# zhiqwang/yolort

Hardware: NVIDIA H100
Metric: images/sec end-to-end (letterbox->NMS) (higher is better)
Workload: dtype f16

## Files before the change

### include/yolort_b200.h

```cpp
#ifndef YOLORT_B200_H
#define YOLORT_B200_H

#include <stddef.h>
#include <stdint.h>

#ifdef __cplusplus
extern "C" {
#endif

#define YB_OK 0
#define YB_ERR_INVALID (-1)
#define YB_ERR_CUDA (-2)
#define YB_ERR_WORKSPACE (-3)

#define YB_U8 0
#define YB_F16 1
#define YB_BF16 2
#define YB_F32 3
#define YB_F8E4M3 4

const char* yb_last_error(void);
int yb_abi_version(void);

typedef struct {
// ... 45 lines not shown
  int32_t level_start;
  int32_t anchors_per_image;
  float stride_px;
  float anchors_px[8];
  float score_thresh;
  int64_t cap_per_image;
  uint64_t* keys;
  void* boxes;
  int32_t* img_count;
  int32_t* img_maxc;
} yb_head_decode;

typedef struct {
  const void* weight;
  const float* bias;
  int32_t Cout, Cout_pad, K_pad;
  int32_t act;
  void* out;
  int32_t out_cstride;
  int32_t own_C;
  const void* extra;
  int32_t extra_C, extra_cstride;
  int32_t store_first;
} yb_conv_chain;

typedef struct {
  int32_t kind;
  int32_t dtype;
  int32_t N, H, W;
  int32_t Cin, in_cstride;
  const void* in;
  int32_t Ho, Wo;
  int32_t Cout, out_cstride;
  void* out;
  int32_t ksize, stride, pad;
  int32_t act;
  const void* weight;
  int32_t Cin_pad, Cout_pad;
  const float* bias;
  const void* residual;
  int32_t res_cstride;
  int32_t reserved;
  const yb_head_decode* decode;
  const yb_conv_chain* chain;
} yb_op_desc;

#define YB_CONV_FORCE_IM2COL 1
#define YB_CONV_BAND_STEM 2
#define YB_CONV_FORCE_PLANES 4
#define YB_CONV_NO_NSPLIT 8
#define YB_CONV_ONE_CTA 16
#define YB_CONV_NO_TAIL_SPLIT 64
#define YB_CONV_PAIR_N64 128
#define YB_CONV_E4M3_F16_OUT 16
#define YB_CONV_E4M3_BF16_OUT 32

int yb_conv_chain_supported(const yb_op_desc* op);

#define YB_CONV_KERNEL_IM2COL 0
#define YB_CONV_KERNEL_PATCH 1
#define YB_CONV_KERNEL_E4M3 2
#define YB_CONV_TILING_ROWS 0
#define YB_CONV_TILING_CLASSIC 1
#define YB_CONV_TILING_WRAP 2
#define YB_CONV_TILING_STRIDE2 3
typedef struct {
  int32_t kernel;
  int32_t block_n;
  int32_t n_tiles;
  int32_t weights_resident;
  int32_t tiles_per_pass;
  int32_t slots;
  int32_t ring;
  int32_t store_cols;
  int32_t store_bufs;
  int32_t groups;
  int32_t resident_ctas;
  int32_t chained;
  int32_t smem_bytes;
  int32_t grid;
  int32_t tiling;
  int32_t m_tiles;
  int32_t work_items;
  int32_t tail_n;
  int32_t tail_tiles;
  int32_t tail_split;
} yb_conv_info;

int yb_conv_config(const yb_op_desc* op, yb_conv_info* info);

typedef struct yb_plan yb_plan;

int yb_plan_create(const yb_op_desc* ops, int n_ops, yb_plan** plan_out);
int yb_plan_run(yb_plan* plan, void* stream);
int yb_plan_run_range(yb_plan* plan, int first, int count, void* stream);
int yb_plan_num_launches(const yb_plan* plan);
int yb_plan_destroy(yb_plan* plan);

#define YB_MAX_LEVELS 4
#define YB_MAX_ANCHORS 4

typedef struct {
  const void* logits;
  int32_t dtype;
  int32_t H, W;
  int64_t stride_n, stride_a, stride_y, stride_x;
// ... 365 lines not shown
```

### yolort_b200/_C.py

```python
import ctypes
import itertools
import math
import os
from typing import Dict, List, Optional, Sequence, Tuple

import torch

_HERE = os.path.dirname(os.path.abspath(__file__))
LIB_PATH = os.environ.get("YB_LIB_PATH") or os.path.join(_HERE, "libyolort_b200.so")

YB_U8, YB_F16, YB_BF16, YB_F32, YB_F8E4M3 = 0, 1, 2, 3, 4
YB_LAYOUT_NCHW, YB_LAYOUT_S2D16 = 0, 1
YB_OP_CONV, YB_OP_SPP_POOL, YB_OP_UPSAMPLE2X, YB_OP_ATTENTION, YB_OP_DWCONV, YB_OP_SE, YB_OP_AVGPOOL = 0, 1, 2, 3, 4, 5, 6
YB_OP_QUANTIZE = 7
YB_ACT_NONE, YB_ACT_SILU, YB_ACT_HARDSWISH, YB_ACT_LEAKY01, YB_ACT_RELU = 0, 1, 2, 3, 4
YB_CONV_FORCE_IM2COL, YB_CONV_BAND_STEM, YB_CONV_FORCE_PLANES, YB_CONV_NO_NSPLIT, YB_CONV_ONE_CTA = 1, 2, 4, 8, 16
YB_CONV_NO_TAIL_SPLIT = 64
YB_CONV_PAIR_N64 = 128
YB_CONV_E4M3_F16_OUT, YB_CONV_E4M3_BF16_OUT = 16, 32
YB_CONV_KERNEL_IM2COL, YB_CONV_KERNEL_PATCH, YB_CONV_KERNEL_E4M3 = 0, 1, 2
PATCH_TILINGS = {1: "classic", 2: "wrap", 3: "stride2"}
YB_MAX_LEVELS, YB_MAX_ANCHORS = 4, 4
NMS_TV_AUTO, NMS_EXACT_PER_CLASS, NMS_OFFSET_TRICK = 0, 1, 2

EXPORTED_SYMBOLS = (
    "yb_last_error",
    "yb_abi_version",
    "yb_letterbox_geometry",
    "yb_letterbox",
    "yb_letterbox_strided",
    "yb_canvas_rescale",
    "yb_scale_coords_params",
    "yb_conv_chain_supported",
    "yb_conv_config",
    "yb_plan_create",
    "yb_plan_run",
    "yb_plan_run_range",
    "yb_plan_num_launches",
    "yb_plan_destroy",
    "yb_decode_nms_workspace_bytes",
    "yb_decode_nms_debug_offset",
    "yb_decode_nms",
    "yb_decode_dense",
    "yb_decode_nms_tta_workspace_bytes",
    "yb_decode_nms_tta",
    "yb_nms_layout",
    "yb_nms_begin",
    "yb_nms_finish",
    "yb_decode_candidates",
    "yb_batched_nms_workspace_bytes",
    "yb_batched_nms",
    "yb_jpeg_parse",
    "yb_jpeg_workspace_bytes",
    "yb_jpeg_decode",
    "yb_coco_append",
    "yb_coco_evaluate_workspace_bytes",
    "yb_coco_evaluate",
    "yb_yolo_loss_workspace_bytes",
    "yb_yolo_loss_layout",
    "yb_yolo_loss_forward",
    "yb_yolo_loss_backward",
    "yb_augment_prepare",
    "yb_augment",
    "yb_augment_sample",
    "yb_v5_augment_prepare",
    "yb_v5_augment",
    "yb_v5_mixup",
    "yb_v5_resize_prepare",
    "yb_v5_resize",
    "yb_v5_compose_prepare",
    "yb_v5_compose",
# ... 1331 lines not shown
```

### yolort_b200/csrc/conv3x3_patch_sm90.cu

```cuda
#include <cstdlib>

#include "common.cuh"
#include "conv_epilogue.cuh"
#include "conv_chain.cuh"
#include "conv_sm90.h"

namespace yb {
namespace {

constexpr int kMaxA = 4, kMaxB = 12;
constexpr int kConsumers = 2;
constexpr int kThreads = 128 * (1 + kConsumers);
constexpr int kStageBufBytes = 128 * 128;
constexpr int kMaxBlockN = 128;
constexpr size_t kSmemBudget = 216 * 1024;
constexpr size_t kStaticSmem = (2 * kMaxA + 2 * kMaxB + 2) * 8 + 2 * kMaxBlockN * 4;
constexpr uint32_t kConsumerBar = 1;

struct TileGeom {
  int tile_h, tile_w;
  int x_step;
  int pitch, patch_h;
  int gpr;
  int sbo_rows;
  int alloc_rows;
};

struct PatchParams {
  int N, H, W;
  int tiles_x, tiles_y, m_tiles, n_tiles, num_tasks;
  int block_n, block_k, chunks;
  int a_slots, b_stages, b_resident;
  int pair;
  int s2;
  int band;
  int ctas;
  int store_cols, store_bufs, bias_len;
  int stage_buf_bytes;
  int kk_last;
  TileGeom tg;
  uint32_t a_bytes, a_stride, b_sub_bytes, b_res_bytes;
  const float* bias;
  EpilogueParams ep;
  ChainParams ch;
};

__device__ __forceinline__ void tma_load_tiled_4d(const void* desc, uint64_t* bar, void* smem_dst, int c, int w,
                                                  int h, int n) {
  asm volatile(
      "cp.async.bulk.tensor.4d.shared::cluster.global.mbarrier::complete_tx::bytes"
      " [%0], [%1, {%3, %4, %5, %6}], [%2];" ::"r"(smem_u32(smem_dst)),
      "l"(reinterpret_cast<uint64_t>(desc)), "r"(smem_u32(bar)), "r"(c), "r"(w), "r"(h), "r"(n)
      : "memory");
}
__device__ __forceinline__ void tma_load_tiled_5d(const void* desc, uint64_t* bar, void* smem_dst, int c, int par, int w,
                                                  int h, int n) {
  asm volatile(
      "cp.async.bulk.tensor.5d.shared::cluster.global.mbarrier::complete_tx::bytes"
      " [%0], [%1, {%3, %4, %5, %6, %7}], [%2];" ::"r"(smem_u32(smem_dst)),
      "l"(reinterpret_cast<uint64_t>(desc)), "r"(smem_u32(bar)), "r"(c), "r"(par), "r"(w), "r"(h), "r"(n)
      : "memory");
}
__device__ __forceinline__ void tma_store_4d(const void* desc, const void* smem_src, int c, int w, int h, int n) {
  asm volatile("cp.async.bulk.tensor.4d.global.shared::cta.bulk_group [%0, {%2, %3, %4, %5}], [%1];" ::"l"(
                   reinterpret_cast<uint64_t>(desc)),
               "r"(smem_u32(smem_src)), "r"(c), "r"(w), "r"(h), "r"(n)
               : "memory");
}

__device__ __forceinline__ void tile_coords(const PatchParams& p, int m_tile, int& n_img, int& y0, int& x0) {
  const int tpi = p.tiles_x * p.tiles_y;
  n_img = m_tile / tpi;
  const int t = m_tile - n_img * tpi;
  const int ty = t / p.tiles_x, tx = t - ty * p.tiles_x;
  y0 = ty * p.tg.tile_h;
  x0 = tx * p.tg.x_step;
}

__device__ __forceinline__ void consumer_sync() { named_bar_sync(kConsumerBar, 128 * kConsumers); }

template <bool kBf16, int kN, bool kPair>
__device__ __forceinline__ void issue_tap(int mode, int tap, int kc, bool first, float* acc, uint32_t a0, uint32_t a1,
                                          uint32_t a_hi, uint32_t b_lo, uint32_t b_hi) {
  for (int k = 0; k < kc; ++k) {
    const bool accum = !(first && k == 0);
    const uint64_t db = desc_lohi(b_lo + 2 * k, b_hi);
    if (mode == 2) {
      wgmma_mma<kBf16, kN>(acc, desc_lohi(((tap % 3) == 1 ? a0 : a1) + 2 * k, a_hi), db, accum);
    } else {
// ... 448 lines not shown
        mbar_wait(&b_full[sb], (kb / p.b_stages) & 1);
        const int dy = tap / 3, dx = tap - dy * 3;
        const uint32_t a_tap = a_lo + static_cast<uint32_t>(dy * p.tg.pitch + dx) * row16;
        const uint32_t b_lo = b_lo0 + static_cast<uint32_t>(sb) * b_step16;
        for (int k = 0; k < kc; ++k)
          wgmma_mma<kBf16, kN>(acc, desc_lohi(a_tap + 2 * k, a_hi), desc_lohi(b_lo + 2 * k, b_hi),
                               !(c == 0 && tap == 0 && k == 0));
        wgmma_commit();
        wgmma_wait<1>();
        if (wg_leader) {
          if (prev_sb >= 0) mbar_arrive(&b_empty[prev_sb]);
          if (prev_sa >= 0) mbar_arrive(&a_empty[prev_sa]);
        }
        prev_sb = sb;
        prev_sa = -1;
      }
      prev_sa = active ? sa : -1;
      ka += cnt;
    }
    wgmma_wait<0>();
    if (wg_leader) {
      mbar_arrive(&b_empty[prev_sb]);
      if (prev_sa >= 0) mbar_arrive(&a_empty[prev_sa]);
    }
    fence_acc<kN / 2>(acc);

    int n_img, y0, x0;
    tile_coords(p, m_first + team, n_img, y0, x0);
#pragma unroll
    for (int rr = 0; rr < 2; ++rr) {
      const int grp = fr.loc[rr] >> 3;
      const int yy = grp / p.tg.gpr, xx = (grp - yy * p.tg.gpr) * 8 + (fr.loc[rr] & 7);
      const int y = y0 + yy, x = x0 + xx;
      fr.ok[rr] = active && yy < p.tg.tile_h && y < p.H && x < p.W;
      fr.row[rr] = (static_cast<long long>(n_img) * p.H + y) * p.W + x;
    }
    uint8_t* team_staging = staging + static_cast<size_t>(team) * p.store_bufs * p.stage_buf_bytes;
#pragma unroll
    for (int c0 = 0; c0 < kN; c0 += 64, ++store_idx) {
      uint8_t* buf = team_staging + (store_idx & 1) * p.stage_buf_bytes;
      epilogue_box<kBf16, kN>(p.ep, acc, c0, 64, s_bias, fr, n0, buf, lane);
      fence_proxy_async_smem();
      if (issuer) tma_store_wait_read<0>();
      named_bar_sync(1 + team, 256);
      if (issuer) {
        if (active && n0 + c0 < p.ep.Cout) tma_store_4d(&tmap_out, buf, n0 + c0, x0, y0, n_img);
        tma_store_commit();
      }
    }
  }
  if (issuer) tma_store_wait_all<0>();
}

}

using PatchKernelFn = void (*)(const CUtensorMap, const CUtensorMap, const CUtensorMap, const CUtensorMap, const CUtensorMap,
                               const CUtensorMap, const PatchParams);

static bool quad_plan(const PatchParams& kp) { return kp.pair == 2 && !kp.s2 && kp.block_n == 128; }

template <bool kBf16>
PatchKernelFn select_patch_kernel_t(const PatchParams& kp) {
  if (quad_plan(kp)) return conv3x3_patch_quad_kernel<kBf16>;
  if (kp.ctas == 2) {
    if (kp.ch.on) return kp.block_n == 32 && kp.ch.n2 == 64 ? conv3x3_patch_kernel<kBf16, 32, 64, 2> : nullptr;
    switch (kp.block_n) {
      case 32: return conv3x3_patch_kernel<kBf16, 32, 0, 2>;
      case 64: return conv3x3_patch_kernel<kBf16, 64, 0, 2>;
      default: return nullptr;
    }
  }
  if (kp.ch.on) {
    if (kp.block_n == 32) return kp.ch.n2 == 64 ? conv3x3_patch_kernel<kBf16, 32, 64, 1> : conv3x3_patch_kernel<kBf16, 32, 128, 1>;
    return kp.ch.n2 == 64 ? conv3x3_patch_kernel<kBf16, 64, 64, 1> : conv3x3_patch_kernel<kBf16, 64, 128, 1>;
  }
  switch (kp.block_n) {
    case 32: return conv3x3_patch_kernel<kBf16, 32, 0, 1>;
    case 64: return conv3x3_patch_kernel<kBf16, 64, 0, 1>;
    default: return conv3x3_patch_kernel<kBf16, 128, 0, 1>;
  }
}
PatchKernelFn select_patch_kernel(const PatchParams& kp) {
  return kp.ep.is_bf16 ? select_patch_kernel_t<true>(kp) : select_patch_kernel_t<false>(kp);
}

namespace {
double classic_eff(int H, int W) {
  const int ty = (H + 15) / 16, tx = (W + 7) / 8;
  return static_cast<double>(H) * W / (static_cast<double>(ty) * tx * 128);
}
double wrap_eff(int H, int W) {
  if (W > 22 || W < 9) return 0.0;
  return static_cast<double>(H) * W / (static_cast<double>((H + 4) / 5) * 128);
}
TileGeom pick_geom(int H, int W, bool allow_wrap, bool s2) {
  TileGeom g;
  if (s2) {
    g.tile_h = 16; g.tile_w = 8; g.x_step = 8; g.pitch = 9; g.patch_h = 33; g.gpr = 1; g.sbo_rows = 18;
    g.alloc_rows = 33 * 9;
  } else if (allow_wrap && wrap_eff(H, W) > classic_eff(H, W)) {
    g.tile_h = 5; g.tile_w = 24; g.x_step = 24; g.pitch = 24; g.patch_h = 7; g.gpr = 3; g.sbo_rows = 8;
    g.alloc_rows = 8 * 24;
  } else {
    g.tile_h = 16; g.tile_w = 8; g.x_step = 8; g.pitch = 10; g.patch_h = 18; g.gpr = 1; g.sbo_rows = 10;
    g.alloc_rows = 18 * 10;
  }
  return g;
}
}

bool patch_conv_eligible(const yb_op_desc& d) {
  if (d.kind != YB_OP_CONV || d.ksize != 3 || d.pad != 1) return false;
  if (d.reserved & YB_CONV_FORCE_IM2COL) return false;
  if (d.stride == 2)
    return (d.reserved & YB_CONV_BAND_STEM) == 0 && d.W % 2 == 0 && d.H % 2 == 0 && classic_eff(d.Ho, d.Wo) >= 0.7 &&
           ((d.Cin <= 64 && d.Cout <= 128) || (d.reserved & YB_CONV_FORCE_PLANES));
// ... 80 lines not shown
        break;
      }
    }
  }
  const size_t avail_ns = budget - staging_ns - 1024 - chain_bytes;
  kp.pair = (!kp.b_resident && !kp.band && !kp.s2 && kp.m_tiles >= 2) ? 2 : 1;
  const int quad_tiles = d.Cout / 128;
  const int quad_tasks = ((kp.m_tiles + 1) / 2) * quad_tiles;
  const int grid_q = quad_tasks < sms ? quad_tasks : sms;
  const bool quad = ctas == 1 && kp.pair == 2 && d.chain == nullptr && d.Cout % 128 == 0 &&
                    !(d.reserved & YB_CONV_PAIR_N64) && grid_q % quad_tiles == 0 && quad_tasks >= sms &&
                    2 * ((quad_tasks + sms - 1) / sms) <= (2 * quad_tasks + sms - 1) / sms;
  const int n_cap = kp.pair == 2 && !quad ? 64 : 128;
  if ((kp.pair == 2 || (kp.s2 && !kp.b_resident)) && block_n > n_cap) {
    n_tiles = (d.Cout + n_cap - 1) / n_cap;
    block_n = mma_n((d.Cout + n_tiles - 1) / n_tiles);
    n_tiles = (d.Cout + block_n - 1) / block_n;
    b_sub = (static_cast<uint32_t>(block_n * kp.block_k * 2) + 1023u) & ~1023u;
    b_total = static_cast<size_t>(9 * kp.chunks) * b_sub;
  }
  YB_REQUIRE(mma_n(block_n) == block_n && block_n <= kMaxBlockN, "patch conv: N tile %d is not a wgmma N", block_n);
  kp.block_n = block_n;
  kp.n_tiles = n_tiles;
  kp.b_sub_bytes = b_sub;
  kp.store_cols = forced_store_cols ? forced_store_cols : ((block_n % 64 == 0) ? 64 : ((block_n % 32 == 0) ? 32 : 16));
  kp.num_tasks = ((kp.m_tiles + kp.pair - 1) / kp.pair) * n_tiles;
  if (kp.band && !(d.Cin_pad == 64 && n_tiles == 1 && kp.store_cols == 64 && d.act < YB_ACT_HARDSWISH &&
                   d.residual == nullptr)) {
    set_error("patch conv: banded stem weights need Cin_pad 64, one N tile with 64-column store boxes, SiLU/linear epilogue");
    return YB_ERR_INVALID;
  }
  if (kp.band && !kp.b_resident) {
    set_error("patch conv: banded stem weights do not fit in shared memory (block_n=%d)", block_n);
    return YB_ERR_INVALID;
  }
  kp.ch.on = 0;
  if (d.chain != nullptr) {
    YB_REQUIRE(kp.b_resident && kp.pair == 1 && !kp.s2 && !kp.band,
               "patch conv: a chained tail needs resident weights and single-tile stride-1 tasks (block_n=%d resident=%d pair=%d)",
               block_n, kp.b_resident, kp.pair);
    YB_REQUIRE(kp.store_cols == block_n && (block_n == 64 || block_n == 32),
               "patch conv: a chained tail needs the first output in one 32- or 64-column box, got block_n=%d", block_n);
    const char* why = chain_setup(d, block_n, n_tiles, kp.store_cols, true, &kp.ch);
    YB_REQUIRE(why == nullptr, "patch conv: chained tail not supported here: %s", why);
    YB_REQUIRE(kp.ch.n2 == 64 || kp.ch.n2 == 128, "patch conv: the tail must have 33-128 output columns, got %d", kp.ch.n2);
    YB_REQUIRE(static_cast<size_t>(kp.ch.w2_chunks) * kp.ch.w2_sub_bytes == chain_bytes, "patch conv: tail weight layout mismatch");
    kp.ch.extra_bytes = static_cast<uint32_t>(tg.tile_w * tg.tile_h) * static_cast<uint32_t>(kp.ch.extra_row_bytes);
  }
  kp.b_res_bytes = kp.b_resident ? static_cast<uint32_t>(b_total) : 0u;
  kp.ep.is_bf16 = d.dtype == YB_BF16;
  if (ctas == 2 && !(kp.b_resident && n_tiles == 1 && kp.pair == 1 && !kp.band && kp.num_tasks >= 2 * sms &&
                     select_patch_kernel(kp) != nullptr))
    return YB_ERR_INVALID;
  if (kp.b_resident) {
    int a_st = static_cast<int>((avail_ns - b_total) / kp.a_stride);
    kp.a_slots = a_st > kMaxA ? kMaxA : a_st;
    kp.b_stages = 1;
  } else if (quad) {
    kp.a_slots = 4;
    staging_ns = 2 * staging;
    const size_t used = 1024 + static_cast<size_t>(kp.a_slots) * kp.a_stride + staging_ns;
    const int b_st = used < kQuadSmemBudget ? static_cast<int>((kQuadSmemBudget - used) / kp.b_sub_bytes) : 0;
    kp.b_stages = b_st > kMaxB ? kMaxB : b_st;
    YB_REQUIRE(kp.b_stages >= 2, "patch conv: not enough shared memory for the weight ring of four consumer warpgroups");
  } else {
    kp.a_slots = (kp.pair == 2 || kp.s2) ? 3 : 2;
    size_t rem = avail - static_cast<size_t>(kp.a_slots) * kp.a_stride;
    if (rem >= static_cast<size_t>(kp.a_stride) + 6 * kp.b_sub_bytes) {
      kp.a_slots += 1;
      rem -= kp.a_stride;
    }
    int b_st = static_cast<int>(rem / kp.b_sub_bytes);
    kp.b_stages = b_st > kMaxB ? kMaxB : b_st;
    if (kp.b_stages < 2) {
      set_error("patch conv: not enough shared memory for the weight ring (block_n=%d)", block_n);
      return YB_ERR_INVALID;
    }
  }
  YB_REQUIRE(kp.a_slots >= 2, "patch conv: fewer than two patch slots fit in shared memory (block_n=%d)", block_n);
  kp.ep.Cout = d.Cout;
  kp.ep.act = d.act;
  kp.ep.residual = d.residual;
  kp.ep.res_cstride = d.res_cstride;
  kp.bias = d.bias;
  const int max_grid = ctas * sms;
  grid = dim3(kp.num_tasks < max_grid ? kp.num_tasks : max_grid, 1, 1);
  YB_REQUIRE(!(kp.b_resident && n_tiles > 1) || grid.x % n_tiles == 0, "patch conv: N-split grid %u not a multiple of %d", grid.x, n_tiles);
  const size_t b_region = kp.b_resident ? kp.b_res_bytes : static_cast<size_t>(kp.b_stages) * kp.b_sub_bytes;
  const size_t smem = static_cast<size_t>(kp.a_slots) * kp.a_stride + b_region + staging_ns + chain_bytes + 1024;
  YB_REQUIRE(smem <= (quad ? kQuadSmemBudget : budget), "patch conv: %zu bytes of shared memory needed, %zu available",
             smem, quad ? kQuadSmemBudget : budget);
  smem_bytes = smem;
  return YB_OK;
}

int patch_conv_config(const yb_op_desc& d, yb_conv_info* info) {
  PatchParams kp;
  dim3 grid;
  size_t smem = 0;
  int rc = conv_validate(d);
  if (rc == YB_OK) rc = patch_conv_configure(d, kp, grid, smem);
  if (rc == YB_OK && info) {
    info->kernel = YB_CONV_KERNEL_PATCH;
    info->block_n = kp.block_n;
    info->n_tiles = kp.n_tiles;
    info->weights_resident = kp.b_resident;
    info->tiles_per_pass = kp.pair;
    info->slots = kp.a_slots;
    info->ring = kp.b_resident ? 0 : kp.b_stages;
    info->store_cols = kp.store_cols;
    info->store_bufs = kp.store_bufs;
    info->groups = quad_plan(kp) ? kQuadConsumers : kConsumers;
    info->resident_ctas = kp.ctas;
    info->chained = kp.ch.on;
    info->smem_bytes = static_cast<int>(smem);
    info->grid = static_cast<int>(grid.x);
    info->tiling = kp.s2 ? YB_CONV_TILING_STRIDE2 : (kp.tg.x_step == 24 ? YB_CONV_TILING_WRAP : YB_CONV_TILING_CLASSIC);
    info->m_tiles = kp.m_tiles;
    info->work_items = kp.num_tasks;
    info->tail_n = kp.ch.n2;
  }
  return rc;
}

struct PatchConvOp final : ConvOp {
  CUtensorMap tmap_a, tmap_b, tmap_out, tmap_w2, tmap_x, tmap_out2;
  PatchParams kp;
  PatchKernelFn fn = nullptr;
  dim3 grid;
  size_t smem_bytes;
  int launch(cudaStream_t stream) const override {
    YB_CHECK_CUDA(launch_pdl(fn, grid, dim3(quad_plan(kp) ? kQuadThreads : kThreads), smem_bytes, stream, tmap_a, tmap_b,
                             tmap_out, tmap_w2, tmap_x, tmap_out2, kp));
    return YB_OK;
  }
};

int patch_conv_create(const yb_op_desc& d, ConvOp** out) {
  PatchConvOp* op = new PatchConvOp();
  PatchParams& kp = op->kp;
  int rc = conv_validate(d);
  if (rc == YB_OK) rc = patch_conv_configure(d, kp, op->grid, op->smem_bytes);
  const TileGeom& tg = kp.tg;
  const CUtensorMapDataType dt = kp.ep.is_bf16 ? CU_TENSOR_MAP_DATA_TYPE_BFLOAT16 : CU_TENSOR_MAP_DATA_TYPE_FLOAT16;
  const uint32_t bk = kp.block_k;
  if (rc == YB_OK && kp.s2) {
    const cuuint64_t dims[5] = {static_cast<cuuint64_t>(d.Cin), 2, static_cast<cuuint64_t>(d.W / 2),
                                static_cast<cuuint64_t>(d.H), static_cast<cuuint64_t>(d.N)};
    const cuuint32_t box[5] = {bk, 1, static_cast<cuuint32_t>(tg.pitch), static_cast<cuuint32_t>(tg.patch_h), 1};
    rc = tmap_tiled(&op->tmap_a, "patch conv stride-2 input planes", dt, d.in, 5, dims, d.in_cstride, box,
                    CU_TENSOR_MAP_L2_PROMOTION_L2_128B);
  } else if (rc == YB_OK) {
    const cuuint64_t dims[4] = {static_cast<cuuint64_t>(d.Cin), static_cast<cuuint64_t>(d.W), static_cast<cuuint64_t>(d.H),
                                static_cast<cuuint64_t>(d.N)};
    const cuuint32_t box[4] = {bk, static_cast<cuuint32_t>(tg.pitch), static_cast<cuuint32_t>(tg.patch_h), 1};
    rc = tmap_tiled(&op->tmap_a, "patch conv input patch", dt, d.in, 4, dims, d.in_cstride, box,
                    CU_TENSOR_MAP_L2_PROMOTION_L2_128B);
  }
  const int ktot = kp.band ? 6 * 64 : 9 * d.Cin_pad;
  if (rc == YB_OK)
    rc = tmap_matrix(&op->tmap_b, "patch conv weights", dt, d.weight, ktot, d.Cout_pad, ktot, bk, kp.block_n,
                     CU_TENSOR_MAP_L2_PROMOTION_L2_256B);
  const cuuint64_t out_px[3] = {static_cast<cuuint64_t>(d.Wo), static_cast<cuuint64_t>(d.Ho), static_cast<cuuint64_t>(d.N)};
  auto out_view = [&](CUtensorMap* map, const char* what, const void* base, int C, int cstride, uint32_t box_c,
                      CUtensorMapL2promotion l2) {
    const cuuint64_t dims[4] = {static_cast<cuuint64_t>(C), out_px[0], out_px[1], out_px[2]};
    const cuuint32_t box[4] = {box_c, static_cast<cuuint32_t>(tg.tile_w), static_cast<cuuint32_t>(tg.tile_h), 1};
    return tmap_tiled(map, what, dt, base, 4, dims, cstride, box, l2);
  };
  if (rc == YB_OK)
    rc = out_view(&op->tmap_out, "patch conv output", d.out, d.Cout, d.out_cstride, kp.store_cols,
                  CU_TENSOR_MAP_L2_PROMOTION_NONE);
  op->tmap_w2 = op->tmap_b;
  op->tmap_x = op->tmap_a;
  op->tmap_out2 = op->tmap_out;
  if (rc == YB_OK && kp.ch.on) {
    const yb_conv_chain& c = *d.chain;
    const uint32_t kc = kp.ch.w2_row_bytes / 2;
    rc = tmap_matrix(&op->tmap_w2, "patch conv chained tail weights", dt, c.weight, c.K_pad, c.Cout_pad, c.K_pad, kc,
                     kp.ch.n2, CU_TENSOR_MAP_L2_PROMOTION_L2_256B);
    if (rc == YB_OK && kp.ch.extra_on)
      rc = out_view(&op->tmap_x, "patch conv chained tail extra operand", c.extra, c.extra_C, c.extra_cstride, kc,
                    CU_TENSOR_MAP_L2_PROMOTION_L2_128B);
    if (rc == YB_OK)
      rc = out_view(&op->tmap_out2, "patch conv chained tail output", c.out, c.Cout, c.out_cstride, 64,
                    CU_TENSOR_MAP_L2_PROMOTION_NONE);
  }
  if (rc == YB_OK) {
    op->fn = select_patch_kernel(kp);
    const bool quad = quad_plan(kp);
    rc = set_smem_attributes(reinterpret_cast<const void*>(op->fn), quad ? kQuadSmemBudget : kSmemBudget, kp.ctas,
                             op->smem_bytes, quad ? kQuadThreads : kThreads, "patch conv");
    if (rc == YB_OK && quad) {
      int per_sm = 0;
      const cudaError_t e = cudaOccupancyMaxActiveBlocksPerMultiprocessor(&per_sm, op->fn, kQuadThreads, op->smem_bytes);
      if (e != cudaSuccess) {
        set_error("patch conv: cudaOccupancyMaxActiveBlocksPerMultiprocessor failed: %s", cudaGetErrorString(e));
        rc = YB_ERR_CUDA;
      } else if (per_sm < 1) {
        set_error("patch conv: the four-warpgroup CTA (%d threads, %zu bytes of shared memory) does not fit on an SM",
                  kQuadThreads, op->smem_bytes);
        rc = YB_ERR_INVALID;
      }
    }
  }
  if (rc != YB_OK) {
    delete op;
    return rc;
  }
  *out = op;
  return YB_OK;
}

}
```

### yolort_b200/csrc/conv_sm90.cu

```cuda
#include <cstdlib>

#include "common.cuh"
#include "conv_sm90.h"
#include "conv_epilogue.cuh"
#include "conv_chain.cuh"
#include "decode_common.cuh"

namespace yb {

namespace {

constexpr int kMaxStages = 12;
__host__ __device__ constexpr int tile_rows(int groups) { return 64 * groups; }
__host__ __device__ constexpr int cta_threads(int groups) { return 128 * (1 + groups); }
__host__ __device__ constexpr int stage_buf_bytes(int groups) { return tile_rows(groups) * 128; }
constexpr int kStageBufs = 2;
constexpr int kMaxBlockN = 256;
constexpr size_t kSmemBudget = 216 * 1024;
constexpr size_t kStaticSmem = (2 * kMaxStages + 2) * 8 + 2 * kMaxBlockN * 4;
constexpr uint32_t kConsumerBar = 1;

struct ConvKernelParams {
  int M, block_n, block_k;
  int ksize, chunks, num_k_iters;
// ... 393 lines not shown
  }
  if (issuer) tma_store_wait_all<0>();
}

using ConvKernelFn = void (*)(const CUtensorMap, const CUtensorMap, const CUtensorMap, const CUtensorMap, const CUtensorMap,
                              const CUtensorMap, const CUtensorMap, const ConvKernelParams);

template <bool kBf16>
ConvKernelFn select_conv_kernel_t(const ConvKernelParams& kp) {
  if (kp.groups == 1) {
    if (kp.ctas != 2 || kp.decode_on || kp.ch.on) return nullptr;
    return kp.block_n == 128 ? conv_wgmma_kernel<kBf16, 128, false, 0, 2, 1> : nullptr;
  }
  if (kp.ctas == 2) {
    if (kp.decode_on) return nullptr;
    if (kp.ch.on) {
      if (kp.block_n != 64) return nullptr;
      return kp.ch.n2 == 32 ? conv_wgmma_kernel<kBf16, 64, false, 32, 2>
                            : (kp.ch.n2 == 64 ? conv_wgmma_kernel<kBf16, 64, false, 64, 2> : nullptr);
    }
    switch (kp.block_n) {
      case 16: return conv_wgmma_kernel<kBf16, 16, false, 0, 2>;
      case 32: return conv_wgmma_kernel<kBf16, 32, false, 0, 2>;
      case 64: return conv_wgmma_kernel<kBf16, 64, false, 0, 2>;
      default: return nullptr;
    }
  }
  if (kp.decode_on) return conv_wgmma_kernel<kBf16, 256, true, 0, 1>;
  if (kp.ch.on) {
    if (kp.block_n == 64)
      return kp.ch.n2 == 32 ? conv_wgmma_kernel<kBf16, 64, false, 32, 1>
                            : (kp.ch.n2 == 64 ? conv_wgmma_kernel<kBf16, 64, false, 64, 1> : conv_wgmma_kernel<kBf16, 64, false, 128, 1>);
    return kp.ch.n2 == 32 ? conv_wgmma_kernel<kBf16, 128, false, 32, 1>
                          : (kp.ch.n2 == 64 ? conv_wgmma_kernel<kBf16, 128, false, 64, 1> : conv_wgmma_kernel<kBf16, 128, false, 128, 1>);
  }
  switch (kp.block_n) {
    case 16: return conv_wgmma_kernel<kBf16, 16, false, 0, 1>;
    case 32: return conv_wgmma_kernel<kBf16, 32, false, 0, 1>;
    case 64: return conv_wgmma_kernel<kBf16, 64, false, 0, 1>;
    case 128: return conv_wgmma_kernel<kBf16, 128, false, 0, 1>;
    default: return conv_wgmma_kernel<kBf16, 256, false, 0, 1>;
  }
}
ConvKernelFn select_conv_kernel(const ConvKernelParams& kp) {
  return kp.ep.is_bf16 ? select_conv_kernel_t<true>(kp) : select_conv_kernel_t<false>(kp);
}

}

static int conv_plan(const yb_op_desc& d, int ctas, int groups, ConvKernelParams& kp, dim3& grid, size_t& smem_bytes);

int conv_validate(const yb_op_desc& d) {
  YB_REQUIRE(d.dtype == YB_F16 || d.dtype == YB_BF16, "conv: dtype must be f16 or bf16");
  YB_REQUIRE((d.reserved & ~(31 | YB_CONV_NO_TAIL_SPLIT | YB_CONV_PAIR_N64)) == 0, "conv: reserved bits 5 and 8 and up must be zero, got 0x%x",
             d.reserved);
  YB_REQUIRE(d.ksize >= 1 && d.ksize <= 7 && d.stride >= 1 && d.stride <= 2, "conv: ksize/stride");
  YB_REQUIRE(d.act >= YB_ACT_NONE && d.act <= YB_ACT_RELU, "conv: unknown activation %d", d.act);
  YB_REQUIRE(d.Cin % 8 == 0 && d.in_cstride % 8 == 0 && d.in_cstride >= d.Cin,
             "conv: Cin/in_cstride must be multiples of 8 (16-byte TMA granularity), got %d/%d", d.Cin,
             d.in_cstride);
  YB_REQUIRE(d.Cout % 8 == 0 && d.out_cstride % 8 == 0 && d.out_cstride >= d.Cout,
             "conv: Cout/out_cstride must be multiples of 8, got %d/%d", d.Cout, d.out_cstride);
  YB_REQUIRE(d.Cin_pad % 16 == 0 && d.Cin_pad >= d.Cin, "conv: Cin_pad must be a multiple of 16");
  YB_REQUIRE(d.Cout_pad % 16 == 0 && d.Cout_pad >= d.Cout, "conv: Cout_pad must be a multiple of 16");
  YB_REQUIRE((reinterpret_cast<uintptr_t>(d.in) & 15) == 0 && (reinterpret_cast<uintptr_t>(d.out) & 15) == 0 &&
                 (reinterpret_cast<uintptr_t>(d.weight) & 15) == 0,
             "conv: tensors must be 16-byte aligned");
  YB_REQUIRE(d.residual == nullptr ||
                 ((reinterpret_cast<uintptr_t>(d.residual) & 15) == 0 && d.res_cstride % 8 == 0),
             "conv: residual alignment");
  int M;
  return conv_rows(d, "conv", &M);
}

static int conv_configure(const yb_op_desc& d, ConvKernelParams& kp, dim3& grid, size_t& smem_bytes) {
  const int rc = conv_validate(d);
  if (rc != YB_OK) return rc;
  YB_REQUIRE(!(d.reserved & YB_CONV_BAND_STEM),
             "conv: banded stem weights (reserved bit 1) need the halo-patch kernel, which this %dx%d map does not qualify for",
             d.H, d.W);
  if (!(d.reserved & YB_CONV_ONE_CTA) &&
      (conv_plan(d, 2, 2, kp, grid, smem_bytes) == YB_OK || conv_plan(d, 2, 1, kp, grid, smem_bytes) == YB_OK))
    return YB_OK;
  return conv_plan(d, 1, 2, kp, grid, smem_bytes);
}

static int conv_plan(const yb_op_desc& d, int ctas, int groups, ConvKernelParams& kp, dim3& grid, size_t& smem_bytes) {
  const int Ho = d.Ho, Wo = d.Wo;
  const size_t budget = ctas == 2 ? smem_per_sm() / 2 - kSmemReservedPerCta - kStaticSmem : kSmemBudget;
  const int block_m = tile_rows(groups);
  kp = ConvKernelParams();
  kp.ctas = ctas;
  kp.groups = groups;
  kp.M = static_cast<int>(static_cast<long long>(d.N) * Ho * Wo);
  kp.ep.Cout = d.Cout;
  const int m_tiles = (kp.M + block_m - 1) / block_m;
  const int sms = num_sms();
  const int m_tiles128 = (kp.M + tile_rows(2) - 1) / tile_rows(2);
  int block_n = conv_block_n(d.Cout, m_tiles128, d.chain != nullptr);
  if (groups == 1) {
    if (block_n != 256 || d.chain != nullptr || m_tiles128 < 3 * sms) return YB_ERR_INVALID;
    block_n = 128;
  }
  if (groups == 2 && ctas == 1 && block_n == 256 && d.chain == nullptr && d.decode == nullptr &&
      !(d.reserved & (YB_CONV_NO_TAIL_SPLIT | YB_CONV_ONE_CTA)) && static_cast<size_t>(d.ksize) * d.ksize * d.Cin_pad * 256 * 2 > 80 * 1024 &&
      m_tiles > sms && m_tiles < 4 * sms && m_tiles % sms != 0) {
    const int n128 = (d.Cout + 127) / 128, r128 = (m_tiles * n128) % sms;
// ... 184 lines not shown
```

Baseline: 7675.

## Add two-team four-warpgroup patch conv kernel for stem and chained convs

Adds a new 3x3 patch-conv kernel in which four consumer warpgroups form two independent teams. Each team processes alternating tiles, sharing one producer warp and the resident weights, with per-team staging buffers and named barriers. It is selected by default for the banded stem (N=128) and for chained 64-column convs when there are enough tasks per SM and shared memory fits. The goal is to overlap one team's epilogue and chain tail with the other team's MMA work and raise tensor-core utilisation. The cost is larger shared-memory use, register caps via setmaxnreg, and a new opt-out flag.

```diff
diff --git a/include/yolort_b200.h b/include/yolort_b200.h
--- a/include/yolort_b200.h
+++ b/include/yolort_b200.h
@@ -121,6 +121,7 @@
 #define YB_CONV_ONE_CTA 16
 #define YB_CONV_NO_TAIL_SPLIT 64
 #define YB_CONV_PAIR_N64 128
+#define YB_CONV_NO_TEAMS 256
 #define YB_CONV_E4M3_F16_OUT 16
 #define YB_CONV_E4M3_BF16_OUT 32
 
diff --git a/yolort_b200/_C.py b/yolort_b200/_C.py
--- a/yolort_b200/_C.py
+++ b/yolort_b200/_C.py
@@ -17,6 +17,7 @@
 YB_CONV_FORCE_IM2COL, YB_CONV_BAND_STEM, YB_CONV_FORCE_PLANES, YB_CONV_NO_NSPLIT, YB_CONV_ONE_CTA = 1, 2, 4, 8, 16
 YB_CONV_NO_TAIL_SPLIT = 64
 YB_CONV_PAIR_N64 = 128
+YB_CONV_NO_TEAMS = 256
 YB_CONV_E4M3_F16_OUT, YB_CONV_E4M3_BF16_OUT = 16, 32
 YB_CONV_KERNEL_IM2COL, YB_CONV_KERNEL_PATCH, YB_CONV_KERNEL_E4M3 = 0, 1, 2
 PATCH_TILINGS = {1: "classic", 2: "wrap", 3: "stride2"}
diff --git a/yolort_b200/csrc/conv3x3_patch_sm90.cu b/yolort_b200/csrc/conv3x3_patch_sm90.cu
--- a/yolort_b200/csrc/conv3x3_patch_sm90.cu
+++ b/yolort_b200/csrc/conv3x3_patch_sm90.cu
@@ -35,6 +35,7 @@
   int s2;
   int band;
   int ctas;
+  int teams;
   int store_cols, store_bufs, bias_len;
   int stage_buf_bytes;
   int kk_last;
@@ -589,16 +590,267 @@
   if (issuer) tma_store_wait_all<0>();
 }
 
+constexpr uint32_t kTeamAllBar = 3;
+constexpr int kTeamMinTasksPerSm = 8;
+constexpr size_t kTeamStaticSmem = (2 * kMaxA + 4) * 8 + 2 * kMaxBlockN * 4;
+constexpr size_t kTeamSmemBudget = 227 * 1024 - kTeamStaticSmem;
+
+template <bool kBf16, int kN, int kN2>
+__global__ void __launch_bounds__(kQuadThreads, 1)
+conv3x3_patch_team_kernel(const __grid_constant__ CUtensorMap tmap_a, const __grid_constant__ CUtensorMap tmap_b,
+                          const __grid_constant__ CUtensorMap tmap_out, const __grid_constant__ CUtensorMap tmap_w2,
+                          const __grid_constant__ CUtensorMap tmap_x, const __grid_constant__ CUtensorMap tmap_out2,
+                          const PatchParams p) {
+  constexpr bool kChain = kN2 != 0;
+  constexpr bool kBand = !kChain;
+  constexpr int kTailChunks = kN2 == 128 ? 2 : 1;
+  static_assert(kBand ? kN == 128 : kN == 64, "team instances: the stem (N = 128) or a chain after N = 64");
+  extern __shared__ uint8_t smem_raw[];
+  __shared__ __align__(8) uint64_t a_full[kMaxA], a_empty[kMaxA];
+  __shared__ __align__(8) uint64_t b_full, w2_full;
+  __shared__ __align__(8) uint64_t x_full[2];
+  __shared__ __align__(16) float s_bias[kN];
+  __shared__ __align__(16) float s_bias2[kChain ? kN2 : 4];
+
+  uint8_t* base = reinterpret_cast<uint8_t*>((reinterpret_cast<uintptr_t>(smem_raw) + 1023) & ~static_cast<uintptr_t>(1023));
+  uint8_t* a_buf = base;
+  uint8_t* b_buf = a_buf + static_cast<size_t>(p.a_slots) * p.a_stride;
+  uint8_t* staging = b_buf + p.b_res_bytes;
+  uint8_t* w2_res = staging + 4 * kStageBufBytes;
+
+  const int warp = threadIdx.x >> 5, lane = threadIdx.x & 31;
+
+  if (threadIdx.x == 0) {
+    tma_prefetch_desc(&tmap_a);
+    tma_prefetch_desc(&tmap_b);
+    tma_prefetch_desc(&tmap_out);
+    for (int s = 0; s < p.a_slots; ++s) {
+      mbar_init(&a_full[s], 1);
+      mbar_init(&a_empty[s], 2);
+    }
+    mbar_init(&b_full, 1);
+    mbar_init(&w2_full, 1);
+    mbar_init(&x_full[0], 1);
+    mbar_init(&x_full[1], 1);
+    mbar_fence_init();
+  }
+  __syncthreads();
+  if (warp != 2) asm volatile("griddepcontrol.wait;" ::: "memory");
+  asm volatile("griddepcontrol.launch_dependents;" ::: "memory");
+  if (warp < 4) asm volatile("setmaxnreg.dec.sync.aligned.u32 24;\n" ::: "memory");
+
+  if (warp == 0) {
+    int ka = 0;
+    for (int task = blockIdx.x; task < p.num_tasks; task += gridDim.x) {
+      int n_img, y0, x0;
+      tile_coords(p, task, n_img, y0, x0);
+      for (int c = 0; c < p.chunks; ++c, ++ka) {
+        const int s = ka % p.a_slots;
+        mbar_wait(&a_empty[s], ((ka / p.a_slots) & 1) ^ 1);
+        if (YB_ELECT()) {
+          mbar_expect_tx(&a_full[s], p.a_bytes);
+          tma_load_tiled_4d(&tmap_a, &a_full[s], a_buf + static_cast<size_t>(s) * p.a_stride, c * p.block_k, x0 - 1,
+                            y0 - 1, n_img);
+        }
+      }
+    }
+    return;
+  }
+  if (warp == 2) {
+    if (lane == 0) {
+      const uint32_t b_bytes = p.block_n * p.block_k * 2;
+      if constexpr (kChain) {
+        tma_prefetch_desc(&tmap_w2);
+        tma_prefetch_desc(&tmap_out2);
+        if (p.ch.extra_on) tma_prefetch_desc(&tmap_x);
+        mbar_expect_tx(&w2_full, p.ch.w2_chunks * p.ch.n2 * p.ch.w2_row_bytes);
+        for (int j = 0; j < p.ch.w2_chunks; ++j)
+          tma_load_2d(&tmap_w2, &w2_full, w2_res + j * p.ch.w2_sub_bytes, j * (p.ch.w2_row_bytes >> 1), 0);
+        const int taps_total = 9 * p.chunks;
+        mbar_expect_tx(&b_full, taps_total * b_bytes);
+        for (int i = 0; i < taps_total; ++i)
+          tma_load_2d(&tmap_b, &b_full, b_buf + static_cast<size_t>(i) * p.b_sub_bytes,
+                      ((i % 9) * p.chunks + i / 9) * p.block_k, 0);
+      } else {
+        mbar_expect_tx(&b_full, 6 * b_bytes);
+        for (int i = 0; i < 6; ++i)
+          tma_load_2d(&tmap_b, &b_full, b_buf + static_cast<size_t>(i) * p.b_sub_bytes, i * p.block_k, 0);
+      }
+    }
+    return;
+  }
+  if (warp < 4) return;
+  asm volatile("setmaxnreg.inc.sync.aligned.u32 112;\n" ::: "memory");
+
+  const int cw = (warp >> 2) - 1;
+  const int team = cw >> 1, half = cw & 1;
+  const int wq = warp & 3;
+  const int ctid = threadIdx.x - 128;
+  const bool issuer = (ctid & 255) == 0;
+  const bool wg_leader = (threadIdx.x & 127) == 0;
+  const uint32_t team_bar = 1 + team;
+  FragRows fr;
+  fr.loc[0] = half * 64 + wq * 16 + (lane >> 2);
+  fr.loc[1] = fr.loc[0] + 8;
+  uint8_t* team_staging = staging + static_cast<size_t>(team) * 2 * kStageBufBytes;
+  float acc[kN / 2];
+
+  for (int i = ctid; i < kN; i += 128 * kQuadConsumers) s_bias[i] = (i < p.bias_len) ? __ldg(p.bias + i) : 0.f;
+  if constexpr (kChain) {
+    for (int i = ctid; i < kN2; i += 128 * kQuadConsumers) s_bias2[i] = (i < p.ch.bias2_len) ? __ldg(p.ch.bias2 + i) : 0.f;
+  }
+  named_bar_sync(kTeamAllBar, 128 * kQuadConsumers);
+  mbar_wait(&b_full, 0);
+  if constexpr (kChain) mbar_wait(&w2_full, 0);
+
+  uint32_t xph = 0;
+  for (int task = blockIdx.x + team * gridDim.x, ka = team * p.chunks; task < p.num_tasks;
+       task += 2 * gridDim.x, ka += 2 * p.chunks) {
+    {
+      const uint32_t row_bytes = p.block_k * 2;
+      const uint32_t sbo = p.tg.sbo_rows * row_bytes;
+      const uint32_t a_wg16 = (8 * sbo * half) >> 4;
+      const uint32_t row16 = row_bytes >> 4;
+      const uint32_t a_hi = desc_hi(row_bytes, sbo);
+      const uint32_t b_hi = desc_hi(row_bytes, 8 * row_bytes);
+      const uint32_t b_lo0 = smem_lo16(b_buf);
+      const uint32_t b_step16 = p.b_sub_bytes >> 4;
+      if constexpr (kChain) {
+#pragma unroll
+        for (int i = 0; i < kN / 2; ++i) acc[i] = 0.f;
+      }
+      for (int c = 0; c < p.chunks; ++c) {
+        const int kq = ka + c;
+        const int sa = kq % p.a_slots;
+        mbar_wait(&a_full[sa], (kq / p.a_slots) & 1);
+        const uint32_t a_lo = smem_lo16(a_buf + static_cast<size_t>(sa) * p.a_stride) + a_wg16;
+        wgmma_fence();
+        if constexpr (kBand) {
+          const uint32_t prow16 = static_cast<uint32_t>(p.tg.pitch) * row16;
+          for (int ky = 0; ky < 3; ++ky) {
+            for (int j = 0; j < 6; ++j) {
+              const uint32_t al = a_lo + ky * prow16 + 6 + 2 * j;
+              const uint32_t b_lo = b_lo0 + static_cast<uint32_t>(ky * 2 + (j >> 2)) * b_step16 + 2 * (j & 3);
+              wgmma_mma<kBf16, kN>(acc, desc_lohi(al, a_hi), desc_lohi(b_lo, b_hi), ky != 0 || j != 0);
+            }
+          }
+        } else {
+          const uint32_t b_lo_chunk = b_lo0 + static_cast<uint32_t>(c * 9) * b_step16;
+          for (int tap = 0; tap < 9; ++tap) {
+            const int dy = tap / 3, dx = tap - dy * 3;
+            const uint32_t a_tap = a_lo + static_cast<uint32_t>(dy * p.tg.pitch + dx) * row16;
+            const uint32_t b_lo = b_lo_chunk + static_cast<uint32_t>(tap) * b_step16;
+#pragma unroll
+            for (int k = 0; k < 4; ++k)
+              wgmma_mma<kBf16, kN>(acc, desc_lohi(a_tap + 2 * k, a_hi), desc_lohi(b_lo + 2 * k, b_hi),
+                                   !(c == 0 && tap == 0 && k == 0));
+          }
+        }
+        wgmma_commit();
+        wgmma_wait<0>();
+        if (wg_leader) mbar_arrive(&a_empty[sa]);
+      }
+    }
+    fence_acc<kN / 2>(acc);
+
+    int n_img, y0, x0;
+    tile_coords(p, task, n_img, y0, x0);
+#pragma unroll
+    for (int rr = 0; rr < 2; ++rr) {
+      const int y = y0 + (fr.loc[rr] >> 3), x = x0 + (fr.loc[rr] & 7);
+      fr.ok[rr] = y < p.H && x < p.W;
+      fr.row[rr] = kBand ? 0 : (static_cast<long long>(n_img) * p.H + y) * p.W + x;
+    }
+    if constexpr (kBand) {
+#pragma unroll
+      for (int c0 = 0; c0 < kN; c0 += 64) {
+        uint8_t* buf = team_staging + (c0 / 64) * kStageBufBytes;
+        epilogue_box<kBf16, kN>(p.ep, acc, c0, 64, s_bias, fr, 0, buf, lane);
+        fence_proxy_async_smem();
+        if (issuer) tma_store_wait_read<0>();
+        named_bar_sync(team_bar, 256);
+        if (issuer) {
+          if (c0 < p.ep.Cout) tma_store_4d(&tmap_out, buf, c0, x0, y0, n_img);
+          tma_store_commit();
+        }
+      }
+    } else {
+      if (issuer) {
+        tma_store_wait_read<0>();
+        if (p.ch.extra_on) {
+          mbar_expect_tx(&x_full[team], p.ch.extra_bytes);
+          tma_load_tiled_4d(&tmap_x, &x_full[team], team_staging + p.ch.own_chunks * kStageBufBytes, 0, x0, y0, n_img);
+        }
+      }
+      named_bar_sync(team_bar, 256);
+      epilogue_box<kBf16, kN>(p.ep, acc, 0, p.store_cols, s_bias, fr, 0, team_staging, lane);
+      fence_proxy_async_smem();
+      named_bar_sync(team_bar, 256);
+      if (issuer) {
+        if (p.ch.store_first) tma_store_4d(&tmap_out, team_staging, 0, x0, y0, n_img);
+        tma_store_commit();
+      }
+      if (p.ch.extra_on) {
+        mbar_wait(&x_full[team], xph);
+        xph ^= 1u;
+      }
+      const uint32_t a2_hi = desc_hi(p.ch.own_row_bytes, 8 * p.ch.own_row_bytes);
+      const uint32_t x_hi = desc_hi(p.ch.extra_row_bytes, 8 * p.ch.extra_row_bytes);
+      const uint32_t w2_lo0 = smem_lo16(w2_res);
+      float acc2[kChain ? kN2 / 2 : 8];
+      wgmma_fence();
+#pragma unroll
+      for (int j = 0; j < kTailChunks; ++j) {
+        const bool own = j == 0;
+        const uint32_t rb = own ? p.ch.own_row_bytes : p.ch.extra_row_bytes;
+        const uint32_t a_lo = smem_lo16(team_staging + j * kStageBufBytes) + ((64 * half * rb) >> 4);
+#pragma unroll
+        for (int k = 0; k < 4; ++k)
+          wgmma_mma<kBf16, kChain ? kN2 : 16>(acc2, desc_lohi(a_lo + 2 * k, own ? a2_hi : x_hi),
+                                              desc_lohi(w2_lo0 + j * (p.ch.w2_sub_bytes >> 4) + 2 * k,
+                                                        desc_hi(p.ch.w2_row_bytes, 8 * p.ch.w2_row_bytes)),
+                                              (j | k) != 0);
+      }
+      wgmma_commit();
+      wgmma_wait<0>();
+      fence_acc<kChain ? kN2 / 2 : 8>(acc2);
+      if (issuer) tma_store_wait_read<0>();
+      named_bar_sync(team_bar, 256);
+      EpilogueParams ep2 = p.ch.ep2;
+      ep2.residual = nullptr;
+#pragma unroll
+      for (int c0 = 0; c0 < (kChain ? kN2 : 16); c0 += 64) {
+        uint8_t* buf = team_staging + ((c0 / 64) & 1) * kStageBufBytes;
+        epilogue_box<kBf16, kChain ? kN2 : 16>(ep2, acc2, c0, 64, s_bias2, fr, 0, buf, lane);
+        fence_proxy_async_smem();
+        if (issuer) tma_store_wait_read<0>();
+        named_bar_sync(team_bar, 256);
+        if (issuer) {
+          if (c0 < p.ch.ep2.Cout) tma_store_4d(&tmap_out2, buf, c0, x0, y0, n_img);
+          tma_store_commit();
+        }
+      }
+    }
+  }
+  if (issuer) tma_store_wait_all<0>();
+}
+
 }
 
 using PatchKernelFn = void (*)(const CUtensorMap, const CUtensorMap, const CUtensorMap, const CUtensorMap, const CUtensorMap,
                                const CUtensorMap, const PatchParams);
 
 static bool quad_plan(const PatchParams& kp) { return kp.pair == 2 && !kp.s2 && kp.block_n == 128; }
+
+static bool four_groups(const PatchParams& kp) { return quad_plan(kp) || kp.teams; }
 
 template <bool kBf16>
 PatchKernelFn select_patch_kernel_t(const PatchParams& kp) {
   if (quad_plan(kp)) return conv3x3_patch_quad_kernel<kBf16>;
+  if (kp.teams) {
+    if (kp.band) return conv3x3_patch_team_kernel<kBf16, 128, 0>;
+    return kp.ch.n2 == 64 ? conv3x3_patch_team_kernel<kBf16, 64, 64> : conv3x3_patch_team_kernel<kBf16, 64, 128>;
+  }
   if (kp.ctas == 2) {
     if (kp.ch.on) return kp.block_n == 32 && kp.ch.n2 == 64 ? conv3x3_patch_kernel<kBf16, 32, 64, 2> : nullptr;
     switch (kp.block_n) {
@@ -785,7 +1037,19 @@
   if (ctas == 2 && !(kp.b_resident && n_tiles == 1 && kp.pair == 1 && !kp.band && kp.num_tasks >= 2 * sms &&
                      select_patch_kernel(kp) != nullptr))
     return YB_ERR_INVALID;
-  if (kp.b_resident) {
+  const bool team_chain = kp.ch.on && block_n == 64 && kp.block_k == 64 && kp.kk_last == 4 && kp.ch.ksteps == 4 &&
+                          kp.ch.w2_chunks == (kp.ch.n2 == 128 ? 2 : 1);
+  const size_t team_fixed = b_total + 2 * staging + chain_bytes + 1024;
+  kp.teams = ctas == 1 && !(d.reserved & (YB_CONV_NO_TEAMS | YB_CONV_PAIR_N64)) && kp.b_resident && n_tiles == 1 &&
+             kp.pair == 1 && !kp.s2 && tg.x_step == 8 && ((kp.band && block_n == 128) || team_chain) &&
+             kp.num_tasks >= kTeamMinTasksPerSm * sms && 2 * kp.chunks <= kMaxA &&
+             team_fixed + 2 * static_cast<size_t>(kp.chunks) * kp.a_stride <= kTeamSmemBudget;
+  if (kp.teams) {
+    const int a_st = static_cast<int>((kTeamSmemBudget - team_fixed) / kp.a_stride);
+    kp.a_slots = (a_st > kMaxA ? kMaxA : a_st) / (2 * kp.chunks) * (2 * kp.chunks);
+    kp.b_stages = 1;
+    staging_ns = 2 * staging;
+  } else if (kp.b_resident) {
     int a_st = static_cast<int>((avail_ns - b_total) / kp.a_stride);
     kp.a_slots = a_st > kMaxA ? kMaxA : a_st;
     kp.b_stages = 1;
@@ -811,6 +1075,8 @@
     }
   }
   YB_REQUIRE(kp.a_slots >= 2, "patch conv: fewer than two patch slots fit in shared memory (block_n=%d)", block_n);
+  YB_REQUIRE(!kp.teams || kp.a_slots % (2 * kp.chunks) == 0, "patch conv: %d patch slots do not divide between two teams",
+             kp.a_slots);
   kp.ep.Cout = d.Cout;
   kp.ep.act = d.act;
   kp.ep.residual = d.residual;
@@ -821,8 +1087,8 @@
   YB_REQUIRE(!(kp.b_resident && n_tiles > 1) || grid.x % n_tiles == 0, "patch conv: N-split grid %u not a multiple of %d", grid.x, n_tiles);
   const size_t b_region = kp.b_resident ? kp.b_res_bytes : static_cast<size_t>(kp.b_stages) * kp.b_sub_bytes;
   const size_t smem = static_cast<size_t>(kp.a_slots) * kp.a_stride + b_region + staging_ns + chain_bytes + 1024;
-  YB_REQUIRE(smem <= (quad ? kQuadSmemBudget : budget), "patch conv: %zu bytes of shared memory needed, %zu available",
-             smem, quad ? kQuadSmemBudget : budget);
+  const size_t cap = quad ? kQuadSmemBudget : (kp.teams ? kTeamSmemBudget : budget);
+  YB_REQUIRE(smem <= cap, "patch conv: %zu bytes of shared memory needed, %zu available", smem, cap);
   smem_bytes = smem;
   return YB_OK;
 }
@@ -843,7 +1109,7 @@
     info->ring = kp.b_resident ? 0 : kp.b_stages;
     info->store_cols = kp.store_cols;
     info->store_bufs = kp.store_bufs;
-    info->groups = quad_plan(kp) ? kQuadConsumers : kConsumers;
+    info->groups = four_groups(kp) ? kQuadConsumers : kConsumers;
     info->resident_ctas = kp.ctas;
     info->chained = kp.ch.on;
     info->smem_bytes = static_cast<int>(smem);
@@ -863,7 +1129,7 @@
   dim3 grid;
   size_t smem_bytes;
   int launch(cudaStream_t stream) const override {
-    YB_CHECK_CUDA(launch_pdl(fn, grid, dim3(quad_plan(kp) ? kQuadThreads : kThreads), smem_bytes, stream, tmap_a, tmap_b,
+    YB_CHECK_CUDA(launch_pdl(fn, grid, dim3(four_groups(kp) ? kQuadThreads : kThreads), smem_bytes, stream, tmap_a, tmap_b,
                              tmap_out, tmap_w2, tmap_x, tmap_out2, kp));
     return YB_OK;
   }
@@ -921,8 +1187,9 @@
   }
   if (rc == YB_OK) {
     op->fn = select_patch_kernel(kp);
-    const bool quad = quad_plan(kp);
-    rc = set_smem_attributes(reinterpret_cast<const void*>(op->fn), quad ? kQuadSmemBudget : kSmemBudget, kp.ctas,
+    const bool quad = four_groups(kp);
+    rc = set_smem_attributes(reinterpret_cast<const void*>(op->fn),
+                             quad_plan(kp) ? kQuadSmemBudget : (kp.teams ? kTeamSmemBudget : kSmemBudget), kp.ctas,
                              op->smem_bytes, quad ? kQuadThreads : kThreads, "patch conv");
     if (rc == YB_OK && quad) {
       int per_sm = 0;
diff --git a/yolort_b200/csrc/conv_sm90.cu b/yolort_b200/csrc/conv_sm90.cu
--- a/yolort_b200/csrc/conv_sm90.cu
+++ b/yolort_b200/csrc/conv_sm90.cu
@@ -469,7 +469,8 @@
 
 int conv_validate(const yb_op_desc& d) {
   YB_REQUIRE(d.dtype == YB_F16 || d.dtype == YB_BF16, "conv: dtype must be f16 or bf16");
-  YB_REQUIRE((d.reserved & ~(31 | YB_CONV_NO_TAIL_SPLIT | YB_CONV_PAIR_N64)) == 0, "conv: reserved bits 5 and 8 and up must be zero, got 0x%x",
+  YB_REQUIRE((d.reserved & ~(31 | YB_CONV_NO_TAIL_SPLIT | YB_CONV_PAIR_N64 | YB_CONV_NO_TEAMS)) == 0,
+             "conv: reserved bits 5 and 9 and up must be zero, got 0x%x",
              d.reserved);
   YB_REQUIRE(d.ksize >= 1 && d.ksize <= 7 && d.stride >= 1 && d.stride <= 2, "conv: ksize/stride");
   YB_REQUIRE(d.act >= YB_ACT_NONE && d.act <= YB_ACT_RELU, "conv: unknown activation %d", d.act);
```

New measurement: 8576, median of 6. 1.12x the previous value.
